# Kolkir/mono_slam_framework

Measured on AMD Instinct MI355X. Metric: frame-pairs/sec (extract+match), higher is better.
Workload: dtype u8; 1 GPU; ORB extract+match, 1280x720 pairs, 1024 pairs/GPU/step resident in HBM, ratio 0.60; pairs_per_gpu=1024, width=1280, height=720, synth_mode=0, overflow_pairs=0, ranks=1, rccl_ranks=0

## Files before the change

mono_slam_framework_amd/csrc/orb_kernels.hip:

```cpp
#include <type_traits>
#include "orb_pipeline.h"

#include <math.h>
#include <stdlib.h>
#include <string.h>

#include "orb_pattern.h"

namespace msf {

constexpr int SW = TW + 2, SH = TH + 2;
constexpr int kTileCandCap = TW * TH / 4;
constexpr int kTileY0 = kEdge;

constexpr uint32_t kStatusOverflow = 1u;

__constant__ __attribute__((aligned(16))) signed char c_pattern[1024];
__constant__ uint32_t c_disc[2 * kDiscTasks];

__device__ __forceinline__ __amdgpu_buffer_rsrc_t uniform_rsrc(const void* p, uint32_t bytes) {
  const unsigned long long v = (unsigned long long)p;
  const uint32_t lo = (uint32_t)__builtin_amdgcn_readfirstlane((int)(uint32_t)v);
  const uint32_t hi = (uint32_t)__builtin_amdgcn_readfirstlane((int)(uint32_t)(v >> 32));
  return __builtin_amdgcn_make_buffer_rsrc((void*)(((unsigned long long)hi << 32) | lo), 0,
// ... 109 lines not shown
        hlow[k] = h1;
      }
      const uint32_t packed = __builtin_amdgcn_perm(v[1], v[0], 0x0c0c0602u) | __builtin_amdgcn_perm(v[3], v[2], 0x06020c0cu);
      if (ry0 + j < rows) *reinterpret_cast<uint32_t*>(dp) = packed;
      dp += L.pitch;
    }
  }
}

constexpr int HX = 16, HY = 4;
constexpr int PW2 = TW + 2 * HX, PH2 = TH + 2 * HY;
constexpr int SCO = 4;
constexpr int GPR = TW / 4 + 2;
constexpr int kList1Cap = 2 * SW * SH;
static_assert(kFastT % 2 == 0, "prefilter constants assume an even FAST threshold (cv::ORB default 20)");

__device__ __forceinline__ uint32_t mbcnt64(unsigned long long m) {
  return __builtin_amdgcn_mbcnt_hi((uint32_t)(m >> 32), __builtin_amdgcn_mbcnt_lo((uint32_t)m, 0u));
}

template <bool BRIGHT, int PITCH = PW2>
__device__ __forceinline__ int fast_score_pol(const uint8_t* p, int tau) {
  constexpr int off[16] = {3 * PITCH + 0,  3 * PITCH + 1,  2 * PITCH + 2,  1 * PITCH + 3,  0 * PITCH + 3, -1 * PITCH + 3,
                           -2 * PITCH + 2, -3 * PITCH + 1, -3 * PITCH + 0, -3 * PITCH - 1, -2 * PITCH - 2, -1 * PITCH - 3,
                           0 * PITCH - 3,  1 * PITCH - 3,  2 * PITCH - 2,  3 * PITCH - 1};
  int q[16];
#pragma unroll
  for (int k = 0; k < 16; k++) q[k] = (int)p[off[k]];
  int m3[16];
#pragma unroll
  for (int k = 0; k < 16; k++)
    m3[k] = BRIGHT ? min(min(q[k], q[(k + 1) & 15]), q[(k + 2) & 15]) : max(max(q[k], q[(k + 1) & 15]), q[(k + 2) & 15]);
  int W = BRIGHT ? -1 : 1000;
#pragma unroll
  for (int k = 0; k < 16; k++) {
    const int w9 = BRIGHT ? min(min(m3[k], m3[(k + 3) & 15]), m3[(k + 6) & 15])
                          : max(max(m3[k], m3[(k + 3) & 15]), m3[(k + 6) & 15]);
    W = BRIGHT ? max(W, w9) : min(W, w9);
  }
  const int v = p[0];
  const int A = BRIGHT ? W - v : v - W;
  return A > tau ? A - 1 : 0;
}

#define MSF_WAVE_SYNC()                                        \
  do {                                                         \
    __builtin_amdgcn_fence(__ATOMIC_RELEASE, "wavefront");     \
    __builtin_amdgcn_wave_barrier();                           \
    __builtin_amdgcn_fence(__ATOMIC_ACQUIRE, "wavefront");     \
  } while (0)

__device__ __forceinline__ uint32_t wave_incl_scan(uint32_t v) {
  v += __builtin_amdgcn_update_dpp(0u, v, 0x111, 0xf, 0xf, false);
  v += __builtin_amdgcn_update_dpp(0u, v, 0x112, 0xf, 0xf, false);
  v += __builtin_amdgcn_update_dpp(0u, v, 0x114, 0xf, 0xf, false);
  v += __builtin_amdgcn_update_dpp(0u, v, 0x118, 0xf, 0xf, false);
  v += __builtin_amdgcn_update_dpp(0u, v, 0x142, 0xa, 0xf, false);
  v += __builtin_amdgcn_update_dpp(0u, v, 0x143, 0xc, 0xf, false);
  return v;
}

__device__ __forceinline__ uint32_t reserve_packed(uint32_t mine, uint32_t* counter, int lane) {
  const uint32_t incl = wave_incl_scan(mine);
  const uint32_t total = __builtin_amdgcn_readlane(incl, 63);
  uint32_t base = 0;
  if (total) {
    if (lane == 0) base = atomicAdd(counter, total);
    base = __builtin_amdgcn_readfirstlane(base);
  }
  return base + incl - mine;
}

constexpr int kFastThreads = 512;

struct FastSmem {
  __attribute__((aligned(16))) uint8_t px[PW2 * PH2];
  __attribute__((aligned(16))) uint8_t sc[PW2 * PH2 + 2 * SCO];
  uint16_t list1[kList1Cap];
  uint2 llist[kTileCandCap];
  uint32_t nbd, lcount, gbase;
};

__global__ __launch_bounds__(256) void k_cand_reset(OrbGeometry g, OrbPrimLists prim, uint2* cmap_rows, int n_frames,
                                                    int dense) {
  const int i = blockIdx.x * 256 + threadIdx.x;
  if (i >= n_frames * kOrbLevels) return;
  const int row = i / kOrbLevels, l = i - row * kOrbLevels;
  if (l >= g.nlevels) { cmap_rows[i] = make_uint2(0u, 0u); return; }
  const OrbLevelInfo& L = g.lv[l];
  cmap_rows[i] = dense ? make_uint2((uint32_t)(g.pool_base + (long long)row * g.cand_total + L.cand_off), (uint32_t)L.cand_cap)
                       : make_uint2((uint32_t)((long long)row * g.prim_total + prim.off[l]), (uint32_t)prim.cap[l]);
}
__device__ __forceinline__ void fast_tile(const OrbGeometry& g, const FrameSrc& src, const uint8_t* pyr, int fi, int l,
                                          int t, int tau, uint32_t* cand_cnt, uint32_t* cand_key, uint8_t* cand_sc,
                                          const uint2* cmap, FastSmem& S_, uint32_t* hist = nullptr,
                                          uint32_t emit_min = 0u) {
  uint8_t* px = S_.px;
  uint8_t* sc = S_.sc;
  uint16_t* list1 = S_.list1;
  uint2* llist = S_.llist;
  const int slot = src.slot0 + fi;
  const OrbLevelInfo L = g.lv[l];
  const int x0 = kTileX0 + (t % L.tiles_x) * TW, y0 = kTileY0 + (t / L.tiles_x) * TH;
  int pitch;
  const uint8_t* img = level_ptr(g, src, pyr, fi, l, &pitch);
  const int tid = threadIdx.x, lane = tid & 63;
  if (tid == 0) { S_.nbd = 0; S_.lcount = 0; }
  const uint32_t lerp_bright = 0x01010101u * (uint32_t)(128 - tau / 2);
  const uint32_t lerp_not_dark = 0x01010101u * (uint32_t)(255 - (254 - tau) / 2);

  for (int i = tid; i < (PW2 / 16) * PH2; i += kFastThreads) {
    const int r = i / (PW2 / 16), c = i % (PW2 / 16);
    const int gx = x0 - HX + 16 * c, gy = y0 - HY + r;
    uint4 v = make_uint4(0u, 0u, 0u, 0u);
    if (gx >= 0 && gx + 16 <= pitch && gy >= 0 && gy < L.h)
      v = *reinterpret_cast<const uint4*>(img + (long long)gy * pitch + gx);
    reinterpret_cast<uint4*>(px)[i] = v;
  }
  for (int i = tid; i < (PW2 * PH2 + 2 * SCO) / 4; i += kFastThreads) reinterpret_cast<uint32_t*>(sc)[i] = 0;
  __syncthreads();

  const uint32_t* T = reinterpret_cast<const uint32_t*>(px);
  constexpr int kLo = kEdge - 1;
  const int txlo = max(-1, kLo - x0), txhi = min(TW, L.w - kLo - 1 - x0);
  const bool inner1 = txlo == -1 && txhi == TW && y0 - 1 >= kLo && y0 + TH < L.h - kLo;
  for (int i0 = 0; i0 < GPR * SH; i0 += kFastThreads) {
    const int i = i0 + tid;
    if (i0 + (tid & ~63) >= GPR * SH) continue;
    const int ic = i < GPR * SH ? i : GPR * SH - 1;
    const int sr = ic / GPR, gq = ic % GPR;
    const int ty = sr - 1, tx0 = 4 * gq - 4;
    const int b = ((ty + HY) * PW2 + tx0 + HX) >> 2;
    const uint32_t C = T[b], Lf = T[b - 1], Rt = T[b + 1];
    const uint32_t U = T[b - 3 * (PW2 / 4)], D = T[b + 3 * (PW2 / 4)];
    const uint32_t W3 = __builtin_amdgcn_alignbyte(C, Lf, 1);
    const uint32_t E3 = __builtin_amdgcn_alignbyte(Rt, C, 3);
    const uint32_t nC = ~C;
    const uint32_t l0 = __builtin_amdgcn_lerp(D, nC, 0), l4 = __builtin_amdgcn_lerp(E3, nC, 0);
    const uint32_t l8 = __builtin_amdgcn_lerp(U, nC, 0), l12 = __builtin_amdgcn_lerp(W3, nC, 0);
    const uint32_t b0 = __builtin_amdgcn_lerp(l0, lerp_bright, 0), b4 = __builtin_amdgcn_lerp(l4, lerp_bright, 0);
    const uint32_t b8 = __builtin_amdgcn_lerp(l8, lerp_bright, 0), b12 = __builtin_amdgcn_lerp(l12, lerp_bright, 0);
    const uint32_t n0 = __builtin_amdgcn_lerp(l0, lerp_not_dark, 0), n4 = __builtin_amdgcn_lerp(l4, lerp_not_dark, 0);
    const uint32_t n8 = __builtin_amdgcn_lerp(l8, lerp_not_dark, 0), n12 = __builtin_amdgcn_lerp(l12, lerp_not_dark, 0);
    uint32_t vm = 0;
    if (inner1) {
      vm = gq == 0 ? 0x80000000u : gq == GPR - 1 ? 0x00000080u : 0x80808080u;
      vm = i < GPR * SH ? vm : 0u;
    } else {
      const int gy = y0 + ty;
      int first = txlo - tx0, last = txhi - tx0;
      first = first < 0 ? 0 : first;
      last = last > 3 ? 3 : last;
      if (i < GPR * SH && gy >= kLo && gy < L.h - kLo && first <= last)
        vm = (0x80808080u << (8 * first)) & (0x80808080u >> (8 * (3 - last)));
    }
    const uint32_t cb = ((b0 | b8) & (b4 | b12)) & vm;
    const uint32_t cd = ~((n0 & n8) | (n4 & n12)) & vm;
    if (__ballot((cb | cd) != 0u) == 0ull) continue;
    const uint32_t e0 = (uint32_t)b << 2;
    const uint32_t slots = reserve_packed(__popc(cb) | (__popc(cd) << 16), &S_.nbd, lane);
    uint32_t k = slots & 0xFFFFu;
    if (cb & 0x80u) list1[k++] = (uint16_t)e0;
    if (cb & 0x8000u) list1[k++] = (uint16_t)(e0 + 1);
    if (cb & 0x800000u) list1[k++] = (uint16_t)(e0 + 2);
    if (cb & 0x80000000u) list1[k++] = (uint16_t)(e0 + 3);
    k = kList1Cap - 1 - (slots >> 16);
    if (cd & 0x80u) list1[k--] = (uint16_t)e0;
    if (cd & 0x8000u) list1[k--] = (uint16_t)(e0 + 1);
    if (cd & 0x800000u) list1[k--] = (uint16_t)(e0 + 2);
// ... 1039 lines not shown
  if (tid < 64) {
    const uint32_t keep = 2u * (uint32_t)L.quota;
    const uint32_t h0 = hist[4 * tid], h1 = hist[4 * tid + 1], h2 = hist[4 * tid + 2], h3 = hist[4 * tid + 3];
    uint32_t above = h0 + h1 + h2 + h3;
#pragma unroll
    for (int o = 1; o < 64; o <<= 1) {
      const uint32_t up = __shfl_down(above, o);
      if (tid + o < 64) above += up;
    }
    above -= h0 + h1 + h2 + h3;
    const uint32_t c3 = above + h3, c2 = c3 + h2, c1 = c2 + h1, c0 = c1 + h0;
    const int mine = c3 >= keep ? 4 * tid + 3 : c2 >= keep ? 4 * tid + 2 : c1 >= keep ? 4 * tid + 1 : c0 >= keep ? 4 * tid : -1;
    const unsigned long long ok = __ballot(mine >= 0);
    uint32_t thr = 0;
    if (n > keep) {
      thr = 256;
      if (keep > 0 && ok) thr = (uint32_t)__shfl(mine, 63 - __builtin_clzll(ok));
    }
    if (tid == 0) thr_s = thr;
  }
  __syncthreads();
  const uint32_t thr = thr_s;
  int pitch;
  const uint8_t* img = level_ptr(g, src, pyr, fi, l, &pitch);
  for (uint32_t i0 = 0; i0 < n; i0 += 16u * nt) {
    const uint32_t i = i0 + 16u * tid;
    uint32_t mask = 0;
    uint4 v = make_uint4(0u, 0u, 0u, 0u);
    if (i < n) {
      v = *reinterpret_cast<const uint4*>(scs + i);
      const uint32_t w[4] = {v.x, v.y, v.z, v.w};
#pragma unroll
      for (int b = 0; b < 16; b++)
        if (i + b < n && ((w[b >> 2] >> (8 * (b & 3))) & 255u) >= thr) mask |= 1u << b;
    }
    if (__ballot(mask != 0u) == 0ull) continue;
    uint32_t k = reserve_packed(__popc(mask), &lcount, tid & 63);
    const uint32_t w[4] = {v.x, v.y, v.z, v.w};
    while (mask) {
      const int b = __ffs(mask) - 1;
      mask &= mask - 1;
      if (k < (uint32_t)kS1Cap)
        out[k] = make_uint4(keys[i + b], 0u, (w[b >> 2] >> (8 * (b & 3))) & 255u, 0u);
      k++;
    }
  }
  __syncthreads();
  const uint32_t kept = !do_harris ? 0u : min(lcount, (uint32_t)kS1Cap);
  for (uint32_t i = tid; i < kept; i += nt) {
    const uint32_t key = out[i].x;
    const float r = harris_at(img, pitch, key & 0xFFFF, key >> 16);
    out[i].y = __float_as_uint(r);
  }
  __syncthreads();
  if (tid == 0) {
    uint32_t m = lcount;
    if (m > (uint32_t)kS1Cap) { atomicOr(&status[slot], kStatusOverflow); m = kS1Cap; }
    s1_cnt[slot * kOrbLevels + l] = m;
  }
}

__global__ __launch_bounds__(256) void k_harris_flat(OrbGeometry g, FrameSrc src, const uint8_t* pyr, HarrisUnits hw,
                                                     const uint32_t* __restrict__ s1_cnt, uint4* s1) {
  const int fi = blockIdx.y, slot = src.slot0 + fi, lane = threadIdx.x & 63;
  const int u = blockIdx.x * 4 + (threadIdx.x >> 6);
  if (u >= hw.base[g.nlevels]) return;
  int l = 0;
#pragma unroll
  for (int i = 1; i < kOrbLevels; i++)
    if (i < g.nlevels && u >= hw.base[i]) l = i;
  const OrbLevelInfo L = g.lv[l];
  const uint32_t kept = min(s1_cnt[slot * kOrbLevels + l], (uint32_t)kS1Cap);
  uint4* out = s1 + (long long)slot * g.s1_total + L.s1_off;
  int pitch;
  const uint8_t* img = level_ptr(g, src, pyr, fi, l, &pitch);
  const uint32_t step = 64u * (uint32_t)hw.n[l];
  for (uint32_t i = 64u * (uint32_t)(u - hw.base[l]) + lane; i < kept; i += step) {
    const uint32_t key = out[i].x;
    out[i].y = __float_as_uint(harris_at(img, pitch, key & 0xFFFF, key >> 16));
  }
}

constexpr int kSelCap = kKpCap;
__global__ __launch_bounds__(256) void k_select(OrbGeometry g, int slot0, const uint32_t* s1_cnt, const uint4* s1,
                                                msf_keypoint* kp, uint32_t* kp_cnt, uint32_t* status) {
  __shared__ uint4 kept[kSelCap];
  constexpr int kRespCap = 4096;
  __shared__ __attribute__((aligned(16))) float resp[kRespCap];
  __shared__ __attribute__((aligned(16))) uint32_t keys[kSelCap];
  __shared__ uint32_t nkept;
  const int slot = slot0 + blockIdx.x, tid = threadIdx.x;
  msf_keypoint* out = kp + (long long)slot * kKpCap;
  uint32_t base = 0;
  bool overflow = false;
  for (int l = 0; l < g.nlevels; l++) {
    const OrbLevelInfo L = g.lv[l];
    const uint32_t n = s1_cnt[slot * kOrbLevels + l];
    const uint4* in = s1 + (long long)slot * g.s1_total + L.s1_off;
    const uint32_t keep = (uint32_t)L.quota;
    if (tid == 0) nkept = 0;
    const bool staged = n > keep && n <= (uint32_t)kRespCap;
    const uint32_t n4 = (n + 3) >> 2;
    if (staged)
      for (uint32_t i = tid; i < 4 * n4; i += 256) resp[i] = i < n ? __uint_as_float(in[i].y) : -INFINITY;
    __syncthreads();
    for (uint32_t i = tid; i < n; i += 256) {
      const uint4 e = in[i];
      bool k = true;
      if (n > keep) {
        const float v = __uint_as_float(e.y);
        uint32_t greater = 0;
        if (staged) {
          const float4* r4 = reinterpret_cast<const float4*>(resp);
          for (uint32_t j = 0; j < n4; j++) {
            const float4 r = r4[j];
            greater += (uint32_t)(r.x > v) + (uint32_t)(r.y > v) + (uint32_t)(r.z > v) + (uint32_t)(r.w > v);
          }
        } else {
          for (uint32_t j = 0; j < n; j++) greater += (__uint_as_float(in[j].y) > v) ? 1u : 0u;
        }
        k = greater < keep;
      }
      if (k) {
        const uint32_t q = atomicAdd(&nkept, 1u);
        if (q < (uint32_t)kSelCap) kept[q] = e;
      }
    }
    __syncthreads();
    uint32_t m = nkept;
    if (m > (uint32_t)kSelCap) { overflow = true; m = kSelCap; }
    if (base + m > (uint32_t)kKpCap) { overflow = true; m = kKpCap - base; }
    const uint32_t m4 = (m + 3) >> 2;
    for (uint32_t i = tid; i < 4 * m4; i += 256) keys[i] = i < m ? kept[i].x : 0xFFFFFFFFu;
    __syncthreads();
    for (uint32_t i = tid; i < m; i += 256) {
      const uint4 e = kept[i];
      uint32_t rank = 0;
      const uint4* k4 = reinterpret_cast<const uint4*>(keys);
      for (uint32_t j = 0; j < m4; j++) {
        const uint4 kk = k4[j];
        rank += (uint32_t)(kk.x < e.x) + (uint32_t)(kk.y < e.x) + (uint32_t)(kk.z < e.x) + (uint32_t)(kk.w < e.x);
      }
      msf_keypoint k;
      k.lx = e.x & 0xFFFF;
      k.ly = e.x >> 16;
      k.x = (float)k.lx * L.scale;
      k.y = (float)k.ly * L.scale;
      k.response = __uint_as_float(e.y);
      k.angle = -1.f;
      k.octave = l;
      k.fast_score = (int)e.z;
      out[base + rank] = k;
    }
    base += m;
    __syncthreads();
  }
  if (tid == 0) {
    kp_cnt[slot] = base;
    if (overflow) atomicOr(&status[slot], kStatusOverflow);
  }
}

__device__ __forceinline__ float fast_atan2_deg(float y, float x) {
  const float k = (float)(180.0 / 3.14159265358979323846);
  const float p1 = 0.9997878412794807f * k, p3 = -0.3258083974640975f * k, p5 = 0.1555786518463281f * k,
              p7 = -0.04432655554792128f * k;
  const float ax = fabsf(x), ay = fabsf(y);
  float a, c, c2;
  if (ax >= ay) {
    c = ay / (ax + (float)2.2204460492503131e-16);
    c2 = c * c;
    a = (((p7 * c2 + p5) * c2 + p3) * c2 + p1) * c;
  } else {
    c = ax / (ay + (float)2.2204460492503131e-16);
    c2 = c * c;
    a = 90.f - (((p7 * c2 + p5) * c2 + p3) * c2 + p1) * c;
  }
  if (x < 0) a = 180.f - a;
  if (y < 0) a = 360.f - a;
  return a;
}

__device__ __forceinline__ void det_sincosf(float t, float* s, float* c) {
  const double x = (double)t;
  const int k = (int)(x * 6.36619772367581382433e-01 + 0.5);
  const double kd = (double)k;
  const double r = (x - kd * 1.57079632673412561417e+00) - kd * 6.07710050650619224932e-11;
  const double z = r * r;
  double p = 1.58969099521155010221e-10;
  p = p * z + -2.50507602534068634195e-08;
  p = p * z + 2.75573137070700676789e-06;
  p = p * z + -1.98412698298579493134e-04;
  p = p * z + 8.33333333332248946124e-03;
  p = p * z + -1.66666666666666324348e-01;
  const double sr = r + (r * z) * p;
  double q = -1.13596475577881948265e-11;
  q = q * z + 2.08757232129817482790e-09;
  q = q * z + -2.75573143513906633035e-07;
  q = q * z + 2.48015872894767294178e-05;
  q = q * z + -1.38888888888741095749e-03;
  q = q * z + 4.16666666666666019037e-02;
  const double cr = (1.0 - 0.5 * z) + (z * z) * q;
  double sv, cv;
  switch (k & 3) {
    case 0: sv = sr; cv = cr; break;
    case 1: sv = cr; cv = -sr; break;
    case 2: sv = -sr; cv = -cr; break;
    default: sv = -cr; cv = sr; break;
  }
  *s = (float)sv;
  *c = (float)cv;
}

constexpr int PR = 22;
constexpr int PD = 2 * PR + 1;
constexpr int PP = 48;
constexpr int HP = 40;
constexpr int HC = 46;

template <bool HALF_UP, bool SUM256>
__global__ __launch_bounds__(256) void k_describe(OrbGeometry g, FrameSrc src, const uint8_t* pyr,
                                                  msf_keypoint* kp, const uint32_t* kp_cnt, uint8_t* desc) {
  __shared__ __attribute__((aligned(16))) uint8_t raw_s[4][PD * PP + 16];
  __shared__ __attribute__((aligned(16))) uint16_t hb_s[4][HP * HC];
  __shared__ uint32_t disc_s[2 * kDiscTasks];
  __shared__ __attribute__((aligned(16))) int pat_s[256];
  const int fi = blockIdx.y, slot = src.slot0 + fi;
  const int wave = __builtin_amdgcn_readfirstlane((int)(threadIdx.x >> 6)), lane = threadIdx.x & 63;
  for (int i = threadIdx.x; i < 2 * kDiscTasks; i += 256) disc_s[i] = c_disc[i];
  pat_s[threadIdx.x] = reinterpret_cast<const int*>(c_pattern)[threadIdx.x];
  __shared__ unsigned long long lvl_base_s[kOrbLevels];
  __shared__ int lvl_pitch_s[kOrbLevels];
  if (threadIdx.x < kOrbLevels) {
    int pt = 0;
    const uint8_t* bp = level_ptr(g, src, pyr, fi, threadIdx.x < g.nlevels ? (int)threadIdx.x : 0, &pt);
    lvl_base_s[threadIdx.x] = (unsigned long long)bp;
    lvl_pitch_s[threadIdx.x] = pt;
  }
  __syncthreads();
  const uint32_t count = min(kp_cnt[slot], (uint32_t)kKpCap);
  uint8_t* raw = raw_s[wave];
  uint16_t* hb = hb_s[wave];
  uint32_t* raw32 = reinterpret_cast<uint32_t*>(raw);
// ... 368 lines not shown
  rq.work_frames = o.work_frames;
  rq.level_size_mul_inv = o.level_size_mul_inv;
  rq.resize_generic = resize_generic_;
  rq.force_tau = force_tau_;
  rq.stream_min_frames = stream_min_frames_;
  OrbPlan plan;
  const std::string err = plan_orb(rq, &plan);
  if (!err.empty()) return err;
  g_ = plan.g;
  prim_ = plan.prim;
  harris_ = plan.harris;
  work_frames_ = plan.work_frames;
  for (int l = 0; l < kOrbLevels; l++) resize_shared_[l] = plan.resize_shared[l];

  const OrbGeometry& g = g_;
  const size_t S = (size_t)max_slots_, Wk = (size_t)work_frames_;
  const size_t total = (size_t)(g.pool_base + (long long)g.pool_entries);
  MSF_HIP_TRY(d_pyr_.reserve(Wk * g.pyr_bytes));
  MSF_HIP_TRY(d_tab_.reserve(plan.tab.size() * sizeof(uint32_t)));
  MSF_HIP_TRY(hipMemcpy(d_tab_, plan.tab.data(), plan.tab.size() * sizeof(uint32_t), hipMemcpyHostToDevice));
  MSF_HIP_TRY(d_cand_cnt_.reserve(Wk * kOrbLevels * sizeof(uint32_t)));
  MSF_HIP_TRY(d_tau_.reserve(2 * Wk * kOrbLevels * sizeof(uint32_t)));
  MSF_HIP_TRY(hipMemset(d_tau_, 0, 2 * Wk * kOrbLevels * sizeof(uint32_t)));
  MSF_HIP_TRY(d_redo_.reserve((1 + Wk * kOrbLevels) * sizeof(uint32_t)));
  MSF_HIP_TRY(d_redo_hist_.reserve(Wk * kOrbLevels * 256 * sizeof(uint32_t)));
  MSF_HIP_TRY(hipMemset(d_redo_hist_, 0, Wk * kOrbLevels * 256 * sizeof(uint32_t)));
  MSF_HIP_TRY(d_redo_thr_.reserve(Wk * kOrbLevels * sizeof(uint32_t)));
  MSF_HIP_TRY(d_qstat_.reserve(Wk * kOrbLevels * kQStat * sizeof(uint32_t)));
  MSF_HIP_TRY(hipMemset(d_qstat_, 0, Wk * kOrbLevels * kQStat * sizeof(uint32_t)));
  MSF_HIP_TRY(d_cand_.reserve(total * sizeof(uint32_t)));
  MSF_HIP_TRY(d_cand_sc_.reserve(total));
  MSF_HIP_TRY(d_cmap_.reserve(Wk * kOrbLevels * sizeof(uint2)));
  MSF_HIP_TRY(hipMemset(d_cmap_, 0, Wk * kOrbLevels * sizeof(uint2)));
  MSF_HIP_TRY(d_walk_abort_.reserve(16));
  MSF_HIP_TRY(hipMemset(d_walk_abort_, 0, 16));
  MSF_HIP_TRY(hipHostMalloc(&h_walk_abort_, 16, hipHostMallocDefault));
  h_walk_abort_[0] = h_walk_abort_[1] = 0u;
  MSF_HIP_TRY(d_s1_cnt_.reserve(Wk * kOrbLevels * sizeof(uint32_t)));
  MSF_HIP_TRY(d_s1_.reserve(Wk * g.s1_total * sizeof(uint4)));
  MSF_HIP_TRY(d_kp_.reserve(S * kKpCap * sizeof(msf_keypoint)));
  MSF_HIP_TRY(d_desc_.reserve(S * kKpCap * 32));
  MSF_HIP_TRY(d_kp_cnt_.reserve(S * sizeof(uint32_t)));
  MSF_HIP_TRY(d_status_.reserve(S * sizeof(uint32_t)));
  MSF_HIP_TRY(d_qres_.reserve((size_t)kSplitMaxPairs * kKpCap * sizeof(uint32_t)));
  MSF_HIP_TRY(d_done_.reserve((size_t)kSplitMaxPairs * sizeof(uint32_t)));
  MSF_HIP_TRY(hipMemset(d_done_, 0, (size_t)kSplitMaxPairs * sizeof(uint32_t)));
  MSF_HIP_TRY(hipMemset(d_kp_cnt_, 0, S * sizeof(uint32_t)));
  MSF_HIP_TRY(hipMemset(d_status_, 0, S * sizeof(uint32_t)));
  MSF_HIP_TRY(hipMemset(d_cand_cnt_, 0, Wk * kOrbLevels * sizeof(uint32_t)));
  MSF_HIP_TRY(hipMemset(d_s1_cnt_, 0, Wk * kOrbLevels * sizeof(uint32_t)));
  MSF_HIP_TRY(hipMemcpyToSymbol(HIP_SYMBOL(c_pattern), k_orb_bit_pattern_31, 1024));
  MSF_HIP_TRY(hipMemcpyToSymbol(HIP_SYMBOL(c_disc), plan.disc.data(), sizeof(uint32_t) * 2 * kDiscTasks));
  if (profile_) {
    for (auto& set : evr_)
      for (auto& e : set.ev) MSF_HIP_TRY(hipEventCreate(&e));
    ev_ok_ = true;
  }
  return "";
}

__global__ __launch_bounds__(256) void k_fill_u32(uint32_t* a, uint32_t* b, uint32_t v, int n) {
  const int i = blockIdx.x * 256 + threadIdx.x;
  if (i < n) { a[i] = v; b[i] = v; }
}

hipError_t OrbPipeline::extract(const FrameSrc& src, int n, hipStream_t st) {
  if (n <= 0) return hipSuccess;
  if (src.slot0 < 0 || src.slot0 + n > max_slots_ || n > work_frames_) return hipErrorInvalidValue;
  last_src_ = src;
  last_n_ = n;
  if (h_walk_abort_ && !walk_per_level_ && __atomic_load_n(&h_walk_abort_[1], __ATOMIC_RELAXED) != 0u) {
    walk_per_level_ = true;
    degraded_note_ = true;
  }
  if (test_stall_frame_ >= 0 && test_stall_calls_++ > 0) test_stall_frame_ = -1;
  if (ev_ok_) ev_begin_call();
  const hipError_t e = extract_range(src, n, st, ev_ok_ ? ev_ : nullptr);
  if (ev_ok_) ev_extract_pending_ = true;
  return e;
}

hipError_t OrbPipeline::extract_range(const FrameSrc& src, int n, hipStream_t st, hipEvent_t* evs) {
  const OrbGeometry& g = g_;
  hipError_t e;
  const ptrdiff_t back = (ptrdiff_t)src.slot0;
  uint8_t* const d_pyr_ = this->d_pyr_ - back * g.pyr_bytes;
  uint32_t* const d_cand_cnt_ = this->d_cand_cnt_ - back * kOrbLevels;
  uint2* const d_cmap_ = this->d_cmap_ - back * kOrbLevels;
  uint32_t* const d_qstat_ = this->d_qstat_ - back * kOrbLevels * kQStat;
  uint32_t* const d_s1_cnt_ = this->d_s1_cnt_ - back * kOrbLevels;
  uint4* const d_s1_ = this->d_s1_ - back * g.s1_total;
  uint32_t* const d_redo_hist_ = this->d_redo_hist_ - back * kOrbLevels * 256;
  uint32_t* const d_redo_thr_ = this->d_redo_thr_ - back * kOrbLevels;
  if ((e = hipMemsetAsync(this->d_cand_cnt_, 0, (size_t)n * kOrbLevels * 4, st))) return e;
  if ((e = hipMemsetAsync(d_status_ + src.slot0, 0, (size_t)n * 4, st))) return e;
  if ((e = hipMemsetAsync(d_redo_, 0, 4, st))) return e;
  if (evs) hipEventRecord(evs[0], st);
  uint32_t* tau = d_tau_ - back * kOrbLevels;
  uint32_t* tau_first = d_tau_ + (ptrdiff_t)work_frames_ * kOrbLevels - back * kOrbLevels;
  const int force_tau = (force_tau_ == 0 && n < stream_min_frames_) ? kFastT : force_tau_;
  const bool dense = force_tau == kFastT;
  if (dense && (long long)n * g.cand_total > (long long)g.pool_entries) return hipErrorInvalidValue;
  hipLaunchKernelGGL(k_cand_reset, dim3((n * kOrbLevels + 255) / 256), dim3(256), 0, st, g, prim_, this->d_cmap_, n, dense ? 1 : 0);
  const int dyn = (fast_two_part_ && force_tau == 0) ? 1 : 0;
  bool fused = fused_ && !dense && g.total_tiles > 0;
  for (int l = 1; l < g.nlevels; l++) fused = fused && g.lv[l].wk_fused != 0;
  auto launch_resize = [&](int l) {
    const OrbLevelInfo& L = g.lv[l];
    const int sw16 = (g.lv[l - 1].w + 16 + 15) & ~15;
    const int groups = (L.w + 3) >> 2;
    int rth = 8;
    const int threads = 256;
    while (rth > 4 && ((rth * 5 + 3) / 4 + 3) * sw16 > 60000) rth -= 4;
    const int lds_rows = (rth * 5 + 3) / 4 + 3;
    const uint32_t magic_n16 = (uint32_t)(0x100000000ull / (uint32_t)(sw16 >> 4)) + 1u;
    const uint32_t magic_groups = groups > 1 ? (uint32_t)(0x100000000ull / (uint32_t)groups) + 1u : 0u;
    hipLaunchKernelGGL(resize_shared_[l] ? k_resize<true> : k_resize<false>, dim3((L.h + rth - 1) / rth, n), dim3(threads),
                       (size_t)lds_rows * sw16 + 8 * kResizeMaxRows, st, g, src, d_pyr_, d_tab_, l, rth, lds_rows, magic_n16,
                       magic_groups);
  };
  auto launch_walk = [&](int l_lo, int l_hi, int chain, int resize_mask, int predict_pct) {
    long long per_frame = 0;
    for (int l = l_lo; l <= l_hi; l++) per_frame += 1 + g.lv[l].wk_nx * g.lv[l].wk_ny;
    const long long wgs = 8ll * ((n + 7) / 8) * per_frame;
    hipLaunchKernelGGL(k_walk, dim3((unsigned)wgs), dim3(64), 0, st, g, src, d_pyr_, d_tab_, tau, tau_first, d_qstat_,
                       d_cand_cnt_, d_cand_, d_cand_sc_, d_cmap_, d_redo_, d_redo_ + 1, d_status_, d_walk_abort_, l_lo, l_hi, n,
                       tau2_margin_pct_, dyn, force_tau, predict_pct, chain, resize_mask, test_stall_frame_);
  };
  last_fused_ = fused;
  last_dense_ = dense;
  if (!dense && g.total_tiles > 0) {
    if ((e = hipMemsetAsync(this->d_qstat_, 0, (size_t)n * kOrbLevels * kQStat * 4, st))) return e;
    if ((e = hipMemsetAsync(d_walk_abort_, 0, 4, st))) return e;
  }
  if (fused) {
    const int mask = (1 << (g.nlevels - 1)) - 1;
    const int predict = dyn ? tau_predict_pct_ : 0;
    if (walk_per_level_) {
      for (int l = 0; l < g.nlevels; l++) launch_walk(l, l, 1, mask, predict);
    } else {
      launch_walk(0, g.nlevels - 1, 1, mask, predict);
    }
    hipMemcpyAsync(h_walk_abort_, d_walk_abort_, 8, hipMemcpyDeviceToHost, st);
    if (evs) hipEventRecord(evs[1], st);
  } else {
    for (int l = 1; l < g.nlevels; l++) launch_resize(l);
    if (evs) hipEventRecord(evs[1], st);
    if (g.total_tiles > 0) {
      if (dense) {
        hipLaunchKernelGGL(k_fill_u32, dim3((n * kOrbLevels + 255) / 256), dim3(256), 0, st, tau + (size_t)src.slot0 * kOrbLevels,
                           tau_first + (size_t)src.slot0 * kOrbLevels, (uint32_t)kFastT, n * kOrbLevels);
        hipLaunchKernelGGL(k_fast, dim3((unsigned)g.total_tiles * (unsigned)n), dim3(kFastThreads), 0, st, g, src, d_pyr_,
                           d_cand_cnt_, d_cand_, d_cand_sc_, d_cmap_);
      } else {
        launch_walk(0, g.nlevels - 1, 0, 0, 0);
      }
    }
  }
  if (g.total_tiles > 0 && !dense) {
    hipLaunchKernelGGL(k_fast_check, dim3((unsigned)n * kOrbLevels), dim3(64), 0, st, g, src.slot0, n, tau, tau_first,
                       d_cand_cnt_, d_cand_sc_, d_cmap_, d_redo_, d_redo_ + 1, d_qstat_);
    long long units = (long long)n * kOrbLevels * g.max_level_tiles;
    unsigned grid = (unsigned)(units < 2048 ? units : 2048);
    grid = (grid + 7u) & ~7u;
    hipLaunchKernelGGL(k_fast_redo, dim3(grid), dim3(kFastThreads), 0, st, g, src, d_pyr_, d_redo_, d_redo_ + 1,
                       g.max_level_tiles, d_cand_cnt_, d_cand_, d_cand_sc_, d_cmap_, d_redo_hist_, (const uint32_t*)nullptr);
    hipLaunchKernelGGL(k_redo_thr, dim3((unsigned)std::min<long long>((long long)n * kOrbLevels, 1024)), dim3(64), 0, st, g,
                       src.slot0, d_redo_, d_redo_ + 1, d_cmap_, d_redo_hist_, d_redo_thr_);
    hipLaunchKernelGGL(k_fast_redo, dim3(grid), dim3(kFastThreads), 0, st, g, src, d_pyr_, d_redo_, d_redo_ + 1,
                       g.max_level_tiles, d_cand_cnt_, d_cand_, d_cand_sc_, d_cmap_, (uint32_t*)nullptr, d_redo_thr_);
  }
  if (evs) hipEventRecord(evs[2], st);
  hipLaunchKernelGGL(k_thr_harris, dim3(g.nlevels, n), dim3(dense ? 256 : 64), 0, st, g, src, d_pyr_,
                     d_cand_cnt_, d_cand_, d_cand_sc_, d_cmap_, d_s1_cnt_, d_s1_, d_status_, dense ? 1 : 0);
  if (!dense) {
    const HarrisUnits& hw = harris_;
    const int nu = hw.base[kOrbLevels];
    hipLaunchKernelGGL(k_harris_flat, dim3((nu + 3) / 4, n), dim3(256), 0, st, g, src, d_pyr_, hw, d_s1_cnt_, d_s1_);
  }
  hipLaunchKernelGGL(k_select, dim3(n), dim3(256), 0, st, g, src.slot0, d_s1_cnt_, d_s1_, d_kp_, d_kp_cnt_,
                     d_status_);
  if (evs) hipEventRecord(evs[3], st);
  {
    int bx = 2048 / n;
    bx = bx < 8 ? 8 : bx > 128 ? 128 : bx;
    auto kd = blur_sum256_ ? k_describe<true, true> : half_up_ ? k_describe<true, false> : k_describe<false, false>;
    hipLaunchKernelGGL(kd, dim3(bx, n), dim3(256), 0, st, g, src, d_pyr_, d_kp_, d_kp_cnt_, d_desc_);
  }
  if (evs) hipEventRecord(evs[4], st);
  return hipGetLastError();
}

static int train_chunk() {
  static const int chunk = [] {
    const char* e = getenv("MSF_ORB_TRAIN_CHUNK");
    const int v = e ? atoi(e) : kTrainChunk;
    return v >= 16 && v <= kTrainChunk ? v : kTrainChunk;
  }();
  return chunk;
}

hipError_t OrbPipeline::set_features(int slot, int n, const msf_keypoint* kp, const uint8_t* desc, hipStream_t st) {
  hipError_t e = hipSuccess;
  if (n > 0) {
    e = hipMemcpyAsync(d_kp_ + (size_t)slot * kKpCap, kp, (size_t)n * sizeof(msf_keypoint), hipMemcpyHostToDevice, st);
    if (e != hipSuccess) return e;
    e = hipMemcpyAsync(d_desc_ + (size_t)slot * kKpCap * 32, desc, (size_t)n * 32, hipMemcpyHostToDevice, st);
    if (e != hipSuccess) return e;
  }
  set_words_[0] = (uint32_t)n;
  set_words_[1] = 0u;
  e = hipMemcpyAsync(d_kp_cnt_ + slot, &set_words_[0], sizeof(uint32_t), hipMemcpyHostToDevice, st);
  if (e != hipSuccess) return e;
  return hipMemcpyAsync(d_status_ + slot, &set_words_[1], sizeof(uint32_t), hipMemcpyHostToDevice, st);
}

hipError_t OrbPipeline::match(int n_pairs, const int32_t* d_slot_a, const int32_t* d_slot_b, float ratio,
                              msf_match* d_out, int cap, int32_t* d_n_out, hipStream_t st, int slot_base, int slot_limit) {
  if (n_pairs <= 0) return hipSuccess;
  const int limit = slot_limit > 0 && slot_limit < max_slots_ ? slot_limit : max_slots_;
  if (ev_ok_ && !ev_extract_pending_) {
    ev_begin_call();
    hipEventRecord(ev_[4], st);
  }
  const int chunk = train_chunk();
  const bool split = n_pairs <= kSplitMaxPairs && d_qres_;
  last_match_form_ = split ? 1 : 2;
  if (split)
    hipLaunchKernelGGL(k_match_split, dim3(kSplitBlocks, n_pairs), dim3(256), 0, st, n_pairs, d_slot_a, d_slot_b, d_kp_,
                       d_kp_cnt_, d_desc_, d_status_, ratio, d_out, cap, d_n_out, chunk, d_qres_, d_done_, slot_base, limit);
  else
    hipLaunchKernelGGL(k_match, dim3(n_pairs), dim3(256), 0, st, n_pairs, d_slot_a, d_slot_b, d_kp_, d_kp_cnt_,
                       d_desc_, d_status_, ratio, d_out, cap, d_n_out, chunk, slot_base, limit);
  if (ev_ok_) {
    hipEventRecord(ev_[5], st);
    EvSet& set = evr_[ev_cur_];
    set.recorded = true;
    set.match_only = !ev_extract_pending_;
    ev_extract_pending_ = false;
  }
  return hipGetLastError();
}

void OrbPipeline::ev_begin_call() {
  if (evr_[ev_cur_].recorded) {
    ev_cur_ = (ev_cur_ + 1) % kEvRing;
    if (evr_[ev_cur_].recorded) ev_harvest(ev_cur_);
  }
  ev_ = evr_[ev_cur_].ev;
}

void OrbPipeline::ev_harvest(int i) {
  EvSet& set = evr_[i];
  if (!set.recorded) return;
  set.recorded = false;
  if (hipEventSynchronize(set.ev[5]) != hipSuccess) return;
  for (int k = set.match_only ? 4 : 0; k < 5; k++) {
    float t = 0.f;
    if (hipEventElapsedTime(&t, set.ev[k], set.ev[k + 1]) == hipSuccess) acc_ms_[k] += t;
  }
  if (set.match_only) acc_match_only_++;
  else acc_full_++;
}

// ... 166 lines not shown
```

Baseline: 161,900 frame-pairs/sec.

## Add all-levels-at-once select kernel for small candidate counts

Adds k_select_batch, which handles every pyramid level of a frame in one pass when the total candidate count fits in a small shared-memory buffer. It stages keys, responses and scores once, then runs the rank-by-response filter and the key-ordered compaction across all levels in parallel instead of looping level by level with barriers. The original k_select now returns early for frames the batch kernel handled, so in non-dense mode it only does the work for frames that overflow the batch cap. The cost is an extra kernel launch plus a re-read of the counts, and the batch path does not set the overflow status bit.

```diff
diff --git a/mono_slam_framework_amd/csrc/orb_kernels.hip b/mono_slam_framework_amd/csrc/orb_kernels.hip
--- a/mono_slam_framework_amd/csrc/orb_kernels.hip
+++ b/mono_slam_framework_amd/csrc/orb_kernels.hip
@@ -1423,14 +1423,22 @@
 }
 
 constexpr int kSelCap = kKpCap;
+constexpr int kSelBatchCap = 1536;
+__device__ __forceinline__ bool select_fits_batch(const OrbGeometry& g, const uint32_t* s1_cnt, int slot) {
+  uint32_t total = 0;
+  for (int l = 0; l < g.nlevels; l++) total += min(s1_cnt[slot * kOrbLevels + l], (uint32_t)kS1Cap);
+  return total <= (uint32_t)kSelBatchCap;
+}
+
 __global__ __launch_bounds__(256) void k_select(OrbGeometry g, int slot0, const uint32_t* s1_cnt, const uint4* s1,
-                                                msf_keypoint* kp, uint32_t* kp_cnt, uint32_t* status) {
+                                                msf_keypoint* kp, uint32_t* kp_cnt, uint32_t* status, int batch) {
   __shared__ uint4 kept[kSelCap];
   constexpr int kRespCap = 4096;
   __shared__ __attribute__((aligned(16))) float resp[kRespCap];
   __shared__ __attribute__((aligned(16))) uint32_t keys[kSelCap];
   __shared__ uint32_t nkept;
   const int slot = slot0 + blockIdx.x, tid = threadIdx.x;
+  if (batch && select_fits_batch(g, s1_cnt, slot)) return;
   msf_keypoint* out = kp + (long long)slot * kKpCap;
   uint32_t base = 0;
   bool overflow = false;
@@ -1500,6 +1508,95 @@
     kp_cnt[slot] = base;
     if (overflow) atomicOr(&status[slot], kStatusOverflow);
   }
+}
+
+__global__ __launch_bounds__(256) __attribute__((amdgpu_waves_per_eu(8))) void k_select_batch(OrbGeometry g, int slot0, const uint32_t* __restrict__ s1_cnt,
+                                                      const uint4* __restrict__ s1, msf_keypoint* kp, uint32_t* kp_cnt) {
+  constexpr int kPad = kSelBatchCap + 4 * kOrbLevels;
+  __shared__ __attribute__((aligned(16))) float resp[kPad];
+  __shared__ __attribute__((aligned(16))) uint32_t keys[kPad];
+  __shared__ uint32_t fast[kPad];
+  __shared__ uint32_t nkept[kOrbLevels];
+  const int slot = slot0 + blockIdx.x, tid = threadIdx.x;
+  uint32_t n[kOrbLevels], off[kOrbLevels + 1];
+  uint32_t total = 0;
+  off[0] = 0;
+#pragma unroll
+  for (int l = 0; l < kOrbLevels; l++) {
+    n[l] = l < g.nlevels ? min(s1_cnt[slot * kOrbLevels + l], (uint32_t)kS1Cap) : 0u;
+    total += n[l];
+    off[l + 1] = off[l] + ((n[l] + 3u) & ~3u);
+  }
+  if (total > (uint32_t)kSelBatchCap) return;
+  if (tid < kOrbLevels) nkept[tid] = 0;
+  const uint4* in = s1 + (long long)slot * g.s1_total;
+  msf_keypoint* out = kp + (long long)slot * kKpCap;
+#define MSF_SEL_LEVEL(p_)                                           \
+  int l = 0;                                                        \
+  uint32_t ol = 0, nl = n[0];                                       \
+  _Pragma("unroll") for (int i_ = 1; i_ < kOrbLevels; i_++)         \
+    if ((p_) >= off[i_]) { l = i_; ol = off[i_]; nl = n[i_]; }
+  for (uint32_t p = tid; p < off[kOrbLevels]; p += 256) {
+    MSF_SEL_LEVEL(p)
+    const uint32_t i = p - ol;
+    uint4 e = make_uint4(0xFFFFFFFFu, __float_as_uint(-INFINITY), 0u, 0u);
+    if (i < nl) e = in[g.lv[l].s1_off + i];
+    keys[p] = e.x;
+    resp[p] = __uint_as_float(e.y);
+    fast[p] = e.z;
+  }
+  __syncthreads();
+  for (uint32_t p = tid; p < off[kOrbLevels]; p += 256) {
+    MSF_SEL_LEVEL(p)
+    if (p - ol >= nl) continue;
+    const uint32_t keep = (uint32_t)g.lv[l].quota;
+    bool k = true;
+    if (nl > keep) {
+      const float v = resp[p];
+      const float4* r4 = reinterpret_cast<const float4*>(resp + ol);
+      uint32_t greater = 0;
+      for (uint32_t j = 0; j < (nl + 3u) >> 2; j++) {
+        const float4 r = r4[j];
+        greater += (uint32_t)(r.x > v) + (uint32_t)(r.y > v) + (uint32_t)(r.z > v) + (uint32_t)(r.w > v);
+      }
+      k = greater < keep;
+    }
+    if (k) atomicAdd(&nkept[l], 1u);
+    else keys[p] = 0xFFFFFFFFu;
+  }
+  __syncthreads();
+  uint32_t base[kOrbLevels + 1];
+  base[0] = 0;
+#pragma unroll
+  for (int l = 0; l < kOrbLevels; l++) base[l + 1] = base[l] + nkept[l];
+  for (uint32_t p = tid; p < off[kOrbLevels]; p += 256) {
+    MSF_SEL_LEVEL(p)
+    const uint32_t key = keys[p];
+    if (key == 0xFFFFFFFFu) continue;
+    uint32_t bl = base[0];
+#pragma unroll
+    for (int i = 1; i < kOrbLevels; i++)
+      if (l == i) bl = base[i];
+    const uint4* k4 = reinterpret_cast<const uint4*>(keys + ol);
+    uint32_t rank = 0;
+    for (uint32_t j = 0; j < (nl + 3u) >> 2; j++) {
+      const uint4 kk = k4[j];
+      rank += (uint32_t)(kk.x < key) + (uint32_t)(kk.y < key) + (uint32_t)(kk.z < key) + (uint32_t)(kk.w < key);
+    }
+    const float scale = g.lv[l].scale;
+    msf_keypoint k;
+    k.lx = key & 0xFFFF;
+    k.ly = key >> 16;
+    k.x = (float)k.lx * scale;
+    k.y = (float)k.ly * scale;
+    k.response = resp[p];
+    k.angle = -1.f;
+    k.octave = l;
+    k.fast_score = (int)fast[p];
+    out[bl + rank] = k;
+  }
+#undef MSF_SEL_LEVEL
+  if (tid == 0) kp_cnt[slot] = base[kOrbLevels];
 }
 
 __device__ __forceinline__ float fast_atan2_deg(float y, float x) {
@@ -2130,8 +2227,10 @@
     const int nu = hw.base[kOrbLevels];
     hipLaunchKernelGGL(k_harris_flat, dim3((nu + 3) / 4, n), dim3(256), 0, st, g, src, d_pyr_, hw, d_s1_cnt_, d_s1_);
   }
+  if (!dense)
+    hipLaunchKernelGGL(k_select_batch, dim3(n), dim3(256), 0, st, g, src.slot0, d_s1_cnt_, d_s1_, d_kp_, d_kp_cnt_);
   hipLaunchKernelGGL(k_select, dim3(n), dim3(256), 0, st, g, src.slot0, d_s1_cnt_, d_s1_, d_kp_, d_kp_cnt_,
-                     d_status_);
+                     d_status_, dense ? 0 : 1);
   if (evs) hipEventRecord(evs[3], st);
   {
     int bx = 2048 / n;
```

Measured after the change: 164,000 frame-pairs/sec (median of 6 runs). +1.3%, better.

## Rewrite keypoint selection as per-level wavefront radix threshold; fold memsets into reset

Applied to the files above, without the earlier changes.

Replaces the per-frame 256-thread top-K selection with a kernel that assigns one wavefront per pyramid level. Each wavefront holds up to 1024 candidates in registers, finds the response cutoff with a bitwise ballot radix search, and compacts and ranks the survivors in shared memory. Frames with more candidates fall back to the old per-level selector in a second kernel, flagged through a sentinel in kp_cnt. Separately, several hipMemsetAsync calls (candidate counts, status, redo counter, walker state, abort word) are folded into the k_cand_reset kernel to cut launch and memset overhead. The cost is an extra launch for the fallback path and more code to keep consistent.

```diff
diff --git a/mono_slam_framework_amd/csrc/orb_kernels.hip b/mono_slam_framework_amd/csrc/orb_kernels.hip
--- a/mono_slam_framework_amd/csrc/orb_kernels.hip
+++ b/mono_slam_framework_amd/csrc/orb_kernels.hip
@@ -215,9 +215,18 @@
 };
 
 __global__ __launch_bounds__(256) void k_cand_reset(OrbGeometry g, OrbPrimLists prim, uint2* cmap_rows, int n_frames,
-                                                    int dense) {
+                                                    int dense, uint32_t* cand_cnt_rows, uint32_t* status_rows,
+                                                    uint32_t* redo_cnt, uint32_t* abort_word, uint4* qstat_rows,
+                                                    uint32_t qstat_u4) {
   const int i = blockIdx.x * 256 + threadIdx.x;
+  for (uint32_t q = (uint32_t)i; q < qstat_u4; q += gridDim.x * 256u) qstat_rows[q] = make_uint4(0u, 0u, 0u, 0u);
+  if (i == 0) {
+    *redo_cnt = 0u;
+    if (qstat_u4) *abort_word = 0u;
+  }
+  if (i < n_frames) status_rows[i] = 0u;
   if (i >= n_frames * kOrbLevels) return;
+  cand_cnt_rows[i] = 0u;
   const int row = i / kOrbLevels, l = i - row * kOrbLevels;
   if (l >= g.nlevels) { cmap_rows[i] = make_uint2(0u, 0u); return; }
   const OrbLevelInfo& L = g.lv[l];
@@ -1423,14 +1432,130 @@
 }
 
 constexpr int kSelCap = kKpCap;
-__global__ __launch_bounds__(256) void k_select(OrbGeometry g, int slot0, const uint32_t* s1_cnt, const uint4* s1,
+constexpr int kSelPer = 16;
+constexpr uint32_t kSelBig = 0xFFFFFFFFu;
+
+__device__ __forceinline__ uint32_t resp_order(uint32_t b) {
+  if (b == 0x80000000u) b = 0u;
+  return (b & 0x80000000u) ? ~b : (b | 0x80000000u);
+}
+
+__global__ __launch_bounds__(64 * kOrbLevels) void k_select(OrbGeometry g, int slot0, const uint32_t* __restrict__ s1_cnt,
+                                                            const uint4* __restrict__ s1, msf_keypoint* kp,
+                                                            uint32_t* kp_cnt, uint32_t* status) {
+  constexpr int kPool = kKpCap + 4 * kOrbLevels;
+  __shared__ __attribute__((aligned(16))) uint32_t keyk[kPool];
+  __shared__ uint16_t idxk[kPool];
+  __shared__ uint32_t cnt[kOrbLevels];
+  const int slot = slot0 + blockIdx.x, lane = threadIdx.x & 63;
+  const int l = __builtin_amdgcn_readfirstlane(threadIdx.x >> 6);
+  bool big = false;
+  for (int j = 0; j < g.nlevels; j++) big = big || s1_cnt[slot * kOrbLevels + j] > 64u * kSelPer;
+  if (big) {
+    if (threadIdx.x == 0) kp_cnt[slot] = kSelBig;
+    return;
+  }
+  const bool live = l < g.nlevels;
+  const OrbLevelInfo& L = g.lv[live ? l : 0];
+  const uint32_t n = live ? s1_cnt[slot * kOrbLevels + l] : 0u;
+  const uint4* in = s1 + (long long)slot * g.s1_total + L.s1_off;
+  const uint32_t keep = (uint32_t)L.quota;
+  const uint32_t kk = (n + 63u) >> 6;
+  uint2 raw[kSelPer];
+#pragma unroll
+  for (int k = 0; k < kSelPer; k++) {
+    const uint32_t i = 64u * k + lane;
+    raw[k] = make_uint2(0xFFFFFFFFu, 0xFFFFFFFFu);
+    if (i < n) raw[k] = *reinterpret_cast<const uint2*>(in + i);
+  }
+  uint32_t key[kSelPer], ord[kSelPer];
+#pragma unroll
+  for (int k = 0; k < kSelPer; k++) {
+    key[k] = raw[k].x;
+    ord[k] = resp_order(raw[k].y);
+  }
+  uint32_t cut = 0u;
+  if (n > keep) {
+    for (int b = 31; b >= 0; b--) {
+      const uint32_t c = cut | (1u << b);
+      uint32_t at_least = 0;
+#pragma unroll
+      for (int k = 0; k < kSelPer; k++)
+        if ((uint32_t)k < kk) at_least += (uint32_t)__popcll(__ballot(ord[k] >= c));
+      if (at_least >= keep) cut = c;
+    }
+  }
+  const bool none = n > keep && keep == 0u;
+  uint32_t kmask = 0, mine = 0;
+#pragma unroll
+  for (int k = 0; k < kSelPer; k++)
+    if ((uint32_t)k < kk) {
+      const bool kept = !none && 64u * k + lane < n && ord[k] >= cut;
+      kmask |= kept ? 1u << k : 0u;
+      mine += (uint32_t)__popcll(__ballot(kept));
+    }
+  if (lane == 0 && live) cnt[l] = mine;
+  __syncthreads();
+  uint32_t base = 0, off = 0, my_base = 0, my_off = 0, m = 0;
+  bool overflow = false;
+  for (int j = 0; j < g.nlevels; j++) {
+    uint32_t mj = cnt[j];
+    if (mj > (uint32_t)kSelCap) { overflow = true; mj = kSelCap; }
+    if (base + mj > (uint32_t)kKpCap) { overflow = true; mj = kKpCap - base; }
+    if (j == l) { my_base = base; my_off = off; m = mj; }
+    base += mj;
+    off += (mj + 3u) & ~3u;
+  }
+  uint32_t run = 0;
+#pragma unroll
+  for (int k = 0; k < kSelPer; k++)
+    if ((uint32_t)k < kk) {
+      const bool kept = (kmask >> k) & 1u;
+      const unsigned long long bal = __ballot(kept);
+      const uint32_t pos = run + __builtin_amdgcn_mbcnt_hi((uint32_t)(bal >> 32), __builtin_amdgcn_mbcnt_lo((uint32_t)bal, 0u));
+      if (kept && pos < m) {
+        keyk[my_off + pos] = key[k];
+        idxk[my_off + pos] = (uint16_t)(64u * k + lane);
+      }
+      run += (uint32_t)__popcll(bal);
+    }
+  if (lane < 4 && m + lane < ((m + 3u) & ~3u)) keyk[my_off + m + lane] = 0xFFFFFFFFu;
+  __syncthreads();
+  msf_keypoint* out = kp + (long long)slot * kKpCap + my_base;
+  const uint4* k4 = reinterpret_cast<const uint4*>(keyk + my_off);
+  const uint32_t m4 = (m + 3u) >> 2;
+  for (uint32_t i = lane; i < m; i += 64) {
+    const uint4 e = in[idxk[my_off + i]];
+    uint32_t rank = 0;
+    for (uint32_t j = 0; j < m4; j++) {
+      const uint4 q = k4[j];
+      rank += (uint32_t)(q.x < e.x) + (uint32_t)(q.y < e.x) + (uint32_t)(q.z < e.x) + (uint32_t)(q.w < e.x);
+    }
+    msf_keypoint k;
+    k.lx = e.x & 0xFFFF;
+    k.ly = e.x >> 16;
+    k.x = (float)k.lx * L.scale;
+    k.y = (float)k.ly * L.scale;
+    k.response = __uint_as_float(e.y);
+    k.angle = -1.f;
+    k.octave = l;
+    k.fast_score = (int)e.z;
+    out[rank] = k;
+  }
+  if (threadIdx.x == 0) {
+    kp_cnt[slot] = base;
+    if (overflow) atomicOr(&status[slot], kStatusOverflow);
+  }
+}
+
+__device__ __forceinline__ void select_by_level(const OrbGeometry& g, int slot, const uint32_t* s1_cnt, const uint4* s1,
                                                 msf_keypoint* kp, uint32_t* kp_cnt, uint32_t* status) {
   __shared__ uint4 kept[kSelCap];
   constexpr int kRespCap = 4096;
   __shared__ __attribute__((aligned(16))) float resp[kRespCap];
   __shared__ __attribute__((aligned(16))) uint32_t keys[kSelCap];
   __shared__ uint32_t nkept;
-  const int slot = slot0 + blockIdx.x, tid = threadIdx.x;
+  const int tid = threadIdx.x;
   msf_keypoint* out = kp + (long long)slot * kKpCap;
   uint32_t base = 0;
   bool overflow = false;
@@ -1499,6 +1624,19 @@
   if (tid == 0) {
     kp_cnt[slot] = base;
     if (overflow) atomicOr(&status[slot], kStatusOverflow);
+  }
+}
+
+constexpr int kSelBigFrames = 4;
+__global__ __launch_bounds__(256) void k_select_big(OrbGeometry g, int slot0, int n_frames, const uint32_t* s1_cnt,
+                                                    const uint4* s1, msf_keypoint* kp, uint32_t* kp_cnt,
+                                                    uint32_t* status) {
+  const int f0 = blockIdx.x * kSelBigFrames, lane = threadIdx.x & 63;
+  unsigned long long marks = __ballot(lane < kSelBigFrames && f0 + lane < n_frames && kp_cnt[slot0 + f0 + lane] == kSelBig);
+  while (marks) {
+    const int j = __ffsll(marks) - 1;
+    marks &= marks - 1;
+    select_by_level(g, slot0 + f0 + j, s1_cnt, s1, kp, kp_cnt, status);
   }
 }
 
@@ -2034,7 +2172,6 @@
 
 hipError_t OrbPipeline::extract_range(const FrameSrc& src, int n, hipStream_t st, hipEvent_t* evs) {
   const OrbGeometry& g = g_;
-  hipError_t e;
   const ptrdiff_t back = (ptrdiff_t)src.slot0;
   uint8_t* const d_pyr_ = this->d_pyr_ - back * g.pyr_bytes;
   uint32_t* const d_cand_cnt_ = this->d_cand_cnt_ - back * kOrbLevels;
@@ -2044,16 +2181,21 @@
   uint4* const d_s1_ = this->d_s1_ - back * g.s1_total;
   uint32_t* const d_redo_hist_ = this->d_redo_hist_ - back * kOrbLevels * 256;
   uint32_t* const d_redo_thr_ = this->d_redo_thr_ - back * kOrbLevels;
-  if ((e = hipMemsetAsync(this->d_cand_cnt_, 0, (size_t)n * kOrbLevels * 4, st))) return e;
-  if ((e = hipMemsetAsync(d_status_ + src.slot0, 0, (size_t)n * 4, st))) return e;
-  if ((e = hipMemsetAsync(d_redo_, 0, 4, st))) return e;
   if (evs) hipEventRecord(evs[0], st);
   uint32_t* tau = d_tau_ - back * kOrbLevels;
   uint32_t* tau_first = d_tau_ + (ptrdiff_t)work_frames_ * kOrbLevels - back * kOrbLevels;
   const int force_tau = (force_tau_ == 0 && n < stream_min_frames_) ? kFastT : force_tau_;
   const bool dense = force_tau == kFastT;
   if (dense && (long long)n * g.cand_total > (long long)g.pool_entries) return hipErrorInvalidValue;
-  hipLaunchKernelGGL(k_cand_reset, dim3((n * kOrbLevels + 255) / 256), dim3(256), 0, st, g, prim_, this->d_cmap_, n, dense ? 1 : 0);
+  {
+    const bool walk = !dense && g.total_tiles > 0;
+    const uint32_t qstat_u4 = walk ? (uint32_t)n * kOrbLevels * (kQStat / 4) : 0u;
+    static_assert(kQStat % 4 == 0, "the walker state is zeroed in 16-byte stores");
+    const unsigned blocks = std::max((unsigned)(n * kOrbLevels + 255) / 256u, (qstat_u4 + 1023u) / 1024u);
+    hipLaunchKernelGGL(k_cand_reset, dim3(blocks), dim3(256), 0, st, g, prim_, this->d_cmap_, n, dense ? 1 : 0,
+                       this->d_cand_cnt_, d_status_ + src.slot0, d_redo_, d_walk_abort_,
+                       reinterpret_cast<uint4*>((uint32_t*)this->d_qstat_), qstat_u4);
+  }
   const int dyn = (fast_two_part_ && force_tau == 0) ? 1 : 0;
   bool fused = fused_ && !dense && g.total_tiles > 0;
   for (int l = 1; l < g.nlevels; l++) fused = fused && g.lv[l].wk_fused != 0;
@@ -2081,10 +2223,6 @@
   };
   last_fused_ = fused;
   last_dense_ = dense;
-  if (!dense && g.total_tiles > 0) {
-    if ((e = hipMemsetAsync(this->d_qstat_, 0, (size_t)n * kOrbLevels * kQStat * 4, st))) return e;
-    if ((e = hipMemsetAsync(d_walk_abort_, 0, 4, st))) return e;
-  }
   if (fused) {
     const int mask = (1 << (g.nlevels - 1)) - 1;
     const int predict = dyn ? tau_predict_pct_ : 0;
@@ -2130,8 +2268,10 @@
     const int nu = hw.base[kOrbLevels];
     hipLaunchKernelGGL(k_harris_flat, dim3((nu + 3) / 4, n), dim3(256), 0, st, g, src, d_pyr_, hw, d_s1_cnt_, d_s1_);
   }
-  hipLaunchKernelGGL(k_select, dim3(n), dim3(256), 0, st, g, src.slot0, d_s1_cnt_, d_s1_, d_kp_, d_kp_cnt_,
+  hipLaunchKernelGGL(k_select, dim3(n), dim3(64 * kOrbLevels), 0, st, g, src.slot0, d_s1_cnt_, d_s1_, d_kp_, d_kp_cnt_,
                      d_status_);
+  hipLaunchKernelGGL(k_select_big, dim3((n + kSelBigFrames - 1) / kSelBigFrames), dim3(256), 0, st, g, src.slot0, n,
+                     d_s1_cnt_, d_s1_, d_kp_, d_kp_cnt_, d_status_);
   if (evs) hipEventRecord(evs[3], st);
   {
     int bx = 2048 / n;
```

New measurement: 164,000 frame-pairs/sec before, 164,700 frame-pairs/sec after, median of 2. About the same (+0.4%).
